# iris-ua/iris_lama

Hardware: AMD Instinct MI355X
Metric: particle-scans/sec (higher is better)
Workload: dtype f64; 1 GPU; PFSlam2D 30 particles, 1080-beam synthetic corridor log (SURVEY.md 8(d)), res 0.05 m, patch 32, l2_max 0.5, GN+Cauchy(0.15), seed 42; particles=30, beams=1080, parallelism=particle-shard x1

## Files before the change

### iris_lama_amd/csrc/lama_kernels.h

```cpp
#pragma once
#include "lama_dev.h"

namespace lama_dev {

constexpr int SM_BLOCK = 256;
constexpr int UM_BLOCK = 64;
#ifdef LAMA_TEST_SMALL_QUEUES
constexpr int LQ_SMALL = LAMA_TEST_SMALL_QUEUES, RQ_SMALL = LAMA_TEST_SMALL_QUEUES / 4;
#else
constexpr int LQ_SMALL = 1024, RQ_SMALL = 256;
#endif
constexpr int LQ_BIG = 8192, RQ_BIG = 2048;
constexpr uint32_t BF_TW_MAX_PARTICLES = 1u << 30;

template <int CTRL, int ROW_MASK>
__device__ __forceinline__ double dpp_add(double v)
{
    const uint64_t u = (uint64_t)__double_as_longlong(v);
    const uint32_t lo = (uint32_t)__builtin_amdgcn_update_dpp(0, (int)(uint32_t)u, CTRL, ROW_MASK, 0xF, false);
    const uint32_t hi = (uint32_t)__builtin_amdgcn_update_dpp(0, (int)(uint32_t)(u >> 32), CTRL, ROW_MASK, 0xF, false);
    return v + __longlong_as_double((long long)(((uint64_t)hi << 32) | lo));
}

template <int NV>
// ... 669 lines not shown
                *cell = o | (vis << 16);
                if (vis == 0) atomicOr((unsigned long long*)(occ_mask + (size_t)slot * 16 + (ci >> 6)), 1ull << (ci & 63));
                }
            }
            const int dslot = coop_slot(dm_dc, dm_dir, dm_count, (int)pv.dm_cap, changed, pidx, ERR_DM_CAP, prm.err);
            bool push = false;
            if (changed && dslot >= 0) {
                const uint64_t bit = 1ull << (ci & 63);
                uint64_t* w = dm_mask + (size_t)dslot * 16 + (ci >> 6);
                if (!(*w & bit)) atomicOr((unsigned long long*)w, (unsigned long long)bit);
                const uint32_t di = (uint32_t)dslot * 1024u + ci;
                const sv_t s = dm_sv[di];
                const bool is_obstacle = (s & SV_VALID) && (s & SV_SQMASK) == 0;
                if (is_hit) {
                    if (!is_obstacle) { dm_sv[di] = (sv_t)(SV_VALID | SV_QUEUED); dm_obs[di] = 0; push = true; }
                } else {
                    if (is_obstacle) { dm_sv[di] = SV_QUEUED; dm_obs[di] = 0; push = true; }
                }
            }
            const unsigned long long pm = __ballot(push);
            if (pm) {
                const unsigned long long pm_hit = (base == 0) ? (pm & 1ull) : 0ull;
                const unsigned long long pm_ray = pm & ~pm_hit;
                if (pm_hit) {
                    if (nl >= prm.qcap) { if (lane == 0) atomicOr(prm.err, ERR_QUEUE); }
                    else { if (push && is_hit) q_lower[nl] = q_entry(0, (int)rx, (int)ry); nl += 1; }
                }
                if (pm_ray) {
                    const int cnt = __popcll(pm_ray);
                    if (nr + (uint32_t)cnt > prm.qcap) { if (lane == 0) atomicOr(prm.err, ERR_QUEUE); }
                    else {
                        if (push && !is_hit) {
                            const int rank = __popcll(pm_ray & ((1ull << lane) - 1ull));
                            q_raise[nr + (uint32_t)rank] = q_entry(0, (int)rx, (int)ry);
                        }
                        nr += (uint32_t)cnt;
                    }
                }
            }
        }
        __builtin_amdgcn_fence(__ATOMIC_SEQ_CST, "wavefront");
    }
    if (lane == 0) {
        prm.counts[2 * p] = dm_count;
        prm.counts[2 * p + 1] = occ_count;
        prm.qsizes[2 * p] = nl;
        prm.qsizes[2 * p + 1] = nr;
        prm.stats[4 * p + 2] += ray_cells;
    }
}

#ifdef LAMA_PROFILE_BF
#ifdef LAMA_PROFILE_BF_COUNT
#define BFT(k) do { (void)tprev; } while (0)
#else
#define BFT(k) do { const uint64_t t_ = __builtin_readcyclecounter(); prof[k] += t_ - tprev; tprev = t_; } while (0)
#endif
#else
#define BFT(k) do {} while (0)
#endif
#ifdef LAMA_PROFILE_BF_MAIN
#define BFT_MAIN(k) BFT(k)
#else
#define BFT_MAIN(k) do {} while (0)
#endif
#ifdef LAMA_PROFILE_BF_FINE
#undef BFT
#undef BFT_MAIN
#define BFT(k) do {} while (0)
#define BFT_MAIN(k) do {} while (0)
#define BFF(k) do { const uint64_t t_ = __builtin_readcyclecounter(); prof[k] += t_ - tprev; tprev = t_; } while (0)
#else
#define BFF(k) do {} while (0)
#endif

constexpr int BF_DUMMY = 8;
template <int LQ, int RQ>
struct BfLds {
    uint64_t pl_e[2][4];
    uint64_t pr_e[2][4];
    uint64_t topq[2];
    uint64_t dummy[2][BF_DUMMY];
    uint32_t pl_n[2];
    uint32_t pr_n[2];
    uint32_t cmd_r;
    uint32_t cmd;
    uint32_t dc[DC_SIZE];
    uint64_t lower[LQ];
    uint64_t raise[RQ];
};
constexpr uint32_t BF_CMD_EXIT = 0xFFFFFFFFu;

__device__ __forceinline__ uint64_t lds_pop_ancestors(int lane)
{
    uint64_t anc = 0;
    if (lane < 63) for (int a = lane; a > 0; a = (a - 1) >> 1) anc |= 1ull << a;
    return anc;
}
__device__ __forceinline__ uint64_t lds_sift_topdown(uint64_t* h, const uint32_t len, const uint32_t H0, const uint64_t value, int lane, uint64_t anc)
{
    const uint32_t vprio = heap_prio(value);
    const uint32_t lim = (len - 1) / 2;
    const int d = 31 - __clz(lane + 1);
    const bool is_left = (lane & 1) != 0;
    uint32_t H = H0;
    uint32_t root_lo = (uint32_t)value, root_hi = (uint32_t)(value >> 32);
    bool stopped = false;
    while (H < lim) {
        const uint32_t idx = (H << d) + (uint32_t)lane;
        const uint32_t left = is_left ? idx : idx - 1;
        const uint32_t parent = (left - 1) >> 1;
        const bool cand = lane >= 1 && lane < 63 && parent < lim;
        const uint32_t la = cand ? left : 1u;
        const uint64_t vl = h[la], vr = h[la + 1];
        const bool take_left = heap_prio(vr) > heap_prio(vl);
        const bool step_to_me = cand && (is_left == take_left);
        const unsigned long long okm = __ballot(step_to_me);
        const bool onpath = cand && (okm & anc) == anc;
        const uint64_t mine = is_left ? vl : vr;
        const bool moves = onpath && !(heap_prio(mine) > vprio);
        const unsigned long long pathm = __ballot(onpath), mvm = __ballot(moves);
        if (moves) h[parent] = mine;
        if (mvm) {
            if (H == 0) {
                const int r1 = (mvm & 2ull) ? 1 : 2;
                root_hi = (uint32_t)__builtin_amdgcn_readlane((int)(uint32_t)(mine >> 32), r1);
                root_lo = (uint32_t)__builtin_amdgcn_readlane((int)(uint32_t)mine, r1);
            }
            const int rel = 63 - __clzll((long long)mvm);
            H = (H << (31 - __clz(rel + 1))) + (uint32_t)rel;
        }
        if (mvm != pathm) { stopped = true; break; }
    }
    LAMA_LOCKSTEP();
    if (!stopped && (len & 1) == 0 && H == (len - 2) / 2) {
        const uint64_t c = h[len - 1];
        const bool up = (uint32_t)__builtin_amdgcn_readfirstlane((int)heap_prio(c)) <= (uint32_t)__builtin_amdgcn_readfirstlane((int)vprio);
        if (up) {
            if (lane == 0) h[H] = c;
            if (H == 0) { root_lo = (uint32_t)c; root_hi = (uint32_t)(c >> 32); }
            H = len - 1;
        }
    }
    if (lane == 0) h[H] = value;
    LAMA_LOCKSTEP();
    return ((uint64_t)root_hi << 32) | root_lo;
}
__device__ __forceinline__ uint64_t lds_pop_topdown(uint64_t* h, uint32_t& size, int lane, uint64_t anc)
{
    --size;
    const uint32_t len = size;
    if (len == 0) return 0;
    return lds_sift_topdown(h, len, 0u, h[len], lane, anc);
}
__device__ __forceinline__ void lds_push(uint64_t* h, uint32_t& size, uint64_t value, bool writer)
{
    uint32_t hole = size++;
    while (hole > 0) {
        const uint32_t parent = (hole - 1) / 2;
        const uint64_t pv = h[parent];
        if (!heap_comp(pv, value)) break;
        if (writer) h[hole] = pv;
        hole = parent;
    }
    if (writer) h[hole] = value;
    LAMA_LOCKSTEP();
}

#ifdef LAMA_WAVE_SIM
struct BufRsrc { uint8_t* base; uint32_t bytes; };
__device__ __forceinline__ BufRsrc buf_make(void* p, uint32_t bytes) { return BufRsrc{(uint8_t*)p, bytes}; }
__device__ __forceinline__ uint32_t buf_load_u16(const BufRsrc& r, uint32_t off) { uint16_t v = 0; if (off <= r.bytes - 2u && off < r.bytes) std::memcpy(&v, r.base + off, 2); return v; }
__device__ __forceinline__ uint32_t buf_load_u32(const BufRsrc& r, uint32_t off) { uint32_t v = 0; if (off <= r.bytes - 4u && off < r.bytes) std::memcpy(&v, r.base + off, 4); return v; }
__device__ __forceinline__ void buf_store_u16(const BufRsrc& r, uint32_t off, uint32_t v) { if (off <= r.bytes - 2u && off < r.bytes) { const uint16_t w = (uint16_t)v; std::memcpy(r.base + off, &w, 2); } }
__device__ __forceinline__ void buf_store_u32(const BufRsrc& r, uint32_t off, uint32_t v) { if (off <= r.bytes - 4u && off < r.bytes) std::memcpy(r.base + off, &v, 4); }
__device__ __forceinline__ void buf_or_u64(const BufRsrc& r, uint32_t off, uint64_t v) { if (off <= r.bytes - 8u && off < r.bytes) { uint64_t w; std::memcpy(&w, r.base + off, 8); w |= v; std::memcpy(r.base + off, &w, 8); } }
__device__ __forceinline__ uint32_t lane_rank(unsigned long long m, int lane) { return (uint32_t)__popcll(m & ((1ull << lane) - 1ull)); }
#else
using BufRsrc = __amdgpu_buffer_rsrc_t;
__device__ __forceinline__ BufRsrc buf_make(void* p, uint32_t bytes) { return __builtin_amdgcn_make_buffer_rsrc(p, 0, (int)bytes, 0x00020000); }
__device__ __forceinline__ uint32_t buf_load_u16(BufRsrc r, uint32_t off) { return (uint32_t)(uint16_t)__builtin_amdgcn_raw_buffer_load_b16(r, (int)off, 0, 0); }
__device__ __forceinline__ uint32_t buf_load_u32(BufRsrc r, uint32_t off) { return (uint32_t)__builtin_amdgcn_raw_buffer_load_b32(r, (int)off, 0, 0); }
__device__ __forceinline__ void buf_store_u16(BufRsrc r, uint32_t off, uint32_t v) { __builtin_amdgcn_raw_buffer_store_b16((unsigned short)v, r, (int)off, 0, 0); }
__device__ __forceinline__ void buf_store_u32(BufRsrc r, uint32_t off, uint32_t v) { __builtin_amdgcn_raw_buffer_store_b32(v, r, (int)off, 0, 0); }
__device__ __forceinline__ void buf_or_u64(BufRsrc r, uint32_t off, uint64_t v) { asm volatile("s_nop 4\n\tbuffer_atomic_or_x2 %0, %1, %2, 0 offen" :: "v"(v), "v"(off), "s"(r) : "memory"); }
__device__ __forceinline__ uint32_t lane_rank(unsigned long long m, int) { return __builtin_amdgcn_mbcnt_hi((uint32_t)(m >> 32), __builtin_amdgcn_mbcnt_lo((uint32_t)m, 0u)); }
#endif
#ifdef LAMA_WIDE_DM
#define buf_load_sv buf_load_u32
#define buf_store_sv buf_store_u32
#else
#define buf_load_sv buf_load_u16
#define buf_store_sv buf_store_u16
#endif
#ifdef LAMA_WAVE_SIM
__device__ __forceinline__ uint32_t opq(uint32_t x) { return x; }
#else
__device__ __forceinline__ uint32_t opq(uint32_t x) { asm("" : "+v"(x)); return x; }
#endif
#ifdef LAMA_WAVE_SIM
__device__ __forceinline__ uint32_t pin(uint32_t x) { return x; }
#else
__device__ __forceinline__ uint32_t pin(uint32_t x) { asm volatile("" : "+v"(x)); return x; }
#endif
__device__ __forceinline__ uint32_t m_lt(uint32_t a, uint32_t b) { return opq((uint32_t)((int32_t)(opq(a) - b) >> 31)); }
__device__ __forceinline__ uint32_t m_le(uint32_t a, uint32_t b) { return ~m_lt(b, a); }
__device__ __forceinline__ uint32_t m_nz(uint32_t v) { return opq((uint32_t)((int32_t)(opq(v) | (0u - v)) >> 31)); }
__device__ __forceinline__ uint32_t m_pos(int32_t a) { return opq((uint32_t)((int32_t)(0u - (uint32_t)opq((uint32_t)a)) >> 31)); }
__device__ __forceinline__ uint32_t m_sel(uint32_t m, uint32_t a, uint32_t b) { return (a & m) | (b & ~m); }
#ifdef LAMA_WAVE_SIM
__device__ __forceinline__ uint32_t bf_mul24(uint32_t a, uint32_t b) { return a * b; }
#else
__device__ __forceinline__ uint32_t bf_mul24(uint32_t a, uint32_t b) { return __umul24(a, b); }
#endif
constexpr uint32_t BUF_OOB = 0x7FFFFFF0u;

template <int NR>
__device__ __forceinline__ void lds_pop_flat(uint64_t* h, uint32_t& size, const int lane, const uint64_t anc, uint64_t* root_out, uint64_t* dummy)
{
    --size;
    const uint32_t len = size;
    if (len == 0) return;
    const uint64_t value = h[len];
    const uint64_t tailc = h[len - 1];
    const uint32_t vprio = heap_prio(value);
    const uint32_t lim = (len - 1) >> 1;
    const int d = 31 - __clz(lane + 1);
    const uint32_t leftm = (lane & 1) ? 0xFFFFFFFFu : 0u;
    const uint32_t innerm = (lane >= 1 && lane < 63) ? 0xFFFFFFFFu : 0u;
    const uint32_t anc_lo = (uint32_t)anc, anc_hi = (uint32_t)(anc >> 32);
    uint32_t H = 0;
    uint32_t go = 0xFFFFFFFFu;
    uint64_t mine0 = 0;
    uint32_t root_child = 0;
    bool root_value = true;
#pragma unroll
    for (int r = 0; r < NR; ++r) {
        if (r > 0 && (go == 0u || ((H << 1) + 1u) >= len)) break;
        const uint32_t idx = (H << d) + (uint32_t)lane;
        const uint32_t lm1 = idx - 2u - leftm;
        const uint32_t parent = lm1 >> 1;
        const uint32_t cand = opq(innerm & go & m_lt(parent, lim));
        const uint32_t la = 1u + (lm1 & cand);
        const uint64_t vl = h[la], vr = h[la + 1];
        const uint32_t pl = (uint32_t)(vl >> 32) >> 16, pr = (uint32_t)(vr >> 32) >> 16;
        const uint32_t take_left = m_lt(pl, pr);
        const uint32_t step = opq(cand & ~(take_left ^ leftm));
        const unsigned long long okm = __ballot(step != 0u);
        const uint32_t offpath = opq((((uint32_t)okm & anc_lo) ^ anc_lo) | (((uint32_t)(okm >> 32) & anc_hi) ^ anc_hi));
        const uint32_t onpath = opq(offpath == 0u ? cand : 0u);
        const uint64_t mine = leftm ? vl : vr;
        const uint32_t pm = leftm ? pl : pr;
        const uint32_t moves = opq(onpath & m_le(pm, vprio));
        const unsigned long long pathm = __ballot(onpath != 0u), mvm = __ballot(moves != 0u);
        LAMA_LOCKSTEP();
        uint64_t* dst = moves ? h + parent : dummy;
        *dst = mine;
        if (r == 0) { mine0 = mine; root_child = opq(((lane == 1 || lane == 2) ? 0xFFFFFFFFu : 0u) & moves); root_value = (mvm & 6ull) == 0ull; }
        const int rel = 63 - __clzll((long long)(mvm | 1ull));
        const uint32_t Hn = (H << (31 - __clz(rel + 1))) + (uint32_t)rel;
        H = mvm ? Hn : H;
        go = (mvm != pathm) ? 0u : go;
        LAMA_LOCKSTEP();
    }
    const bool up = go != 0u && (len & 1u) == 0u && H == (len - 2) / 2 && heap_prio(tailc) <= vprio;
    if (__builtin_expect(up, 0)) {
        if (lane == 0) { h[H] = tailc; if (H == 0) *root_out = tailc; }
        root_value = root_value && H != 0;
        H = len - 1;
        LAMA_LOCKSTEP();
    }
    {
        const uint32_t l0 = lane == 0 ? 0xFFFFFFFFu : 0u, l3 = (lane == 3 && root_value) ? 0xFFFFFFFFu : 0u;
        uint64_t* dst = l0 ? h + H : ((l3 | root_child) ? root_out : dummy);
        const uint64_t v = root_child ? mine0 : value;
        *dst = v;
    }
    LAMA_LOCKSTEP();
}

__device__ __forceinline__ void lds_push_flat(uint64_t* heap, uint32_t& n, const uint64_t* ent, const uint32_t* cnt_p, const int lane, uint64_t* dummy)
{
    const uint32_t l4 = (uint32_t)lane & 3u;
    const uint64_t entry = ent[l4];
    const uint32_t pos = n + l4;
    const uint32_t pprio = heap_prio(heap[n >= 4 ? (pos - 1) / 2 : 0]);
    const uint32_t cnt_v = *cnt_p;
    const bool mine = (uint32_t)lane < cnt_v;
    const bool up = mine && pprio > heap_prio(entry);
    const unsigned long long upm = __ballot(up);
    const uint32_t cnt = (uint32_t)__builtin_amdgcn_readfirstlane((int)cnt_v);
    if (cnt == 0) return;
    if (__builtin_expect(n >= 4 && upm == 0ull, 1)) {
        uint64_t* dst = mine ? heap + pos : dummy;
        *dst = entry;
        n += cnt;
        LAMA_LOCKSTEP();
        return;
    }
    #pragma unroll 1
    for (uint32_t i = 0; i < cnt; ++i) lds_push(heap, n, ent[i], lane == 0);
}

__device__ __forceinline__ void lds_push_flat_n(uint64_t* heap, uint32_t& n, const uint64_t* ent, const uint32_t cnt, const int lane, uint64_t* dummy)
{
    if (cnt == 0) return;
    const uint32_t l4 = (uint32_t)lane & 3u;
    const uint64_t entry = ent[l4];
    const uint32_t pos = n + l4;
    const uint32_t pprio = heap_prio(heap[n >= 4 ? (pos - 1) / 2 : 0]);
    const bool mine = (uint32_t)lane < cnt;
    const bool up = mine && pprio > heap_prio(entry);
    const unsigned long long upm = __ballot(up);
    if (n >= 4 && upm == 0ull) {
        uint64_t* dst = mine ? heap + pos : dummy;
        *dst = entry;
        n += cnt;
        LAMA_LOCKSTEP();
        return;
    }
    #pragma unroll 1
    for (uint32_t i = 0; i < cnt; ++i) lds_push(heap, n, ent[i], lane == 0);
}

__device__ __forceinline__ bool lds_push_list(uint64_t* heap, uint32_t& n, const uint64_t* ent, const uint32_t cnt, int lane)
{
    if (!cnt) return false;
    const uint32_t l4 = (uint32_t)lane & 3u;
    const uint64_t entry = ent[l4];
    const uint32_t pos = n + l4;
    if (n >= 4) {
        const uint32_t pprio = heap_prio(heap[(pos - 1) / 2]);
        const bool mine = (uint32_t)lane < cnt;
        const bool up = mine && pprio > heap_prio(entry);
        if (__ballot(up) == 0) {
            if (mine) heap[pos] = entry;
            n += cnt;
            LAMA_LOCKSTEP();
            return true;
        }
    }
    #pragma unroll 1
    for (uint32_t i = 0; i < cnt; ++i) lds_push(heap, n, ent[i], lane == 0);
    return false;
}

#ifdef LAMA_WAVE_SIM
__device__ __forceinline__ void lds_barrier() { __syncthreads(); }
#else
__device__ __forceinline__ void lds_barrier() { asm volatile("s_waitcnt lgkmcnt(0)\n\ts_barrier" ::: "memory"); }
#endif

#ifdef LAMA_WAVE_SIM
__device__ __forceinline__ uint64_t uniform_u64(uint64_t v) { return v; }
#else
__device__ __forceinline__ uint64_t uniform_u64(uint64_t v)
{
    return ((uint64_t)(uint32_t)__builtin_amdgcn_readfirstlane((int)(uint32_t)(v >> 32)) << 32) | (uint32_t)__builtin_amdgcn_readfirstlane((int)(uint32_t)v);
}
#endif

__device__ __forceinline__ void bf_hand_over(const DevParams& prm, int p, bool from_resume)
{
    prm.slow[p] = 1;
    if (!from_resume) prm.slow_list[atomicAdd(prm.slow_n, 1u)] = (uint32_t)p;
}

template <int LQ_LDS, int RQ_LDS, bool RESUME, bool TW>
__device__ __forceinline__ void bf_particle(const DevParams& prm, const int p_any, BfLds<LQ_LDS, RQ_LDS>& sh)
{
    const int p = __builtin_amdgcn_readfirstlane(p_any);
    if (!RESUME && prm.heavy != nullptr && (prm.heavy[p] != 0 || (prm.early != nullptr && prm.early[p] != 0))) return;
    const uint32_t handed = RESUME ? prm.slow[p] : 1u;
    const int lane = threadIdx.x & 63;
    const int tid = threadIdx.x, nthreads = TW ? 2 * UM_BLOCK : UM_BLOCK;
    const PV pv = pview_w(prm, p);
    int16_t* dir = pv.dm_dir;
    sv_t* sv = pv.dm_sv;
    uint32_t* obs = pv.dm_obs;
    uint64_t* mask = pv.dm_mask;
    const uint32_t dm_cap = pv.dm_cap;
    uint64_t* g_lower = prm.q_lower + (size_t)p * prm.qcap;
    uint64_t* g_raise = prm.q_raise + (size_t)p * prm.qcap;
    int count = uload_i32(prm.counts + 2 * p);
    const uint64_t nlr = uload_u64(prm.qsizes + 2 * p);
    uint32_t nl = (uint32_t)nlr, nr = (uint32_t)(nlr >> 32);
    if (RESUME && TW) __syncthreads(); else LAMA_LOCKSTEP();
    if (RESUME && handed == 0) return;
    if (tid == 0) prm.slow[p] = 0;
    if (nl == 0 && nr == 0) return;
    if (nl + 4 > (uint32_t)LQ_LDS || nr + 4 > (uint32_t)RQ_LDS) { if (tid == 0) bf_hand_over(prm, p, RESUME); return; }

    for (int k = tid; k < DC_SIZE; k += nthreads) sh.dc[k] = DC_EMPTY;
    for (uint32_t k = tid; k < nl; k += nthreads) sh.lower[k] = g_lower[k];
    for (uint32_t k = tid; k < nr; k += nthreads) sh.raise[k] = g_raise[k];
    __syncthreads();
    const uint64_t anc = lds_pop_ancestors(lane);
    constexpr uint32_t LOWER_CAP = RESUME ? (uint32_t)LQ_LDS : (uint32_t)(LQ_LDS + RQ_LDS);
#ifndef LAMA_WAVE_SIM
    if (TW) { if (tid >= UM_BLOCK) __builtin_amdgcn_s_setprio(0); else __builtin_amdgcn_s_setprio(3); }
#endif
    if (TW && tid >= UM_BLOCK) {
        __syncthreads();
        uint32_t hnl = (uint32_t)__builtin_amdgcn_readfirstlane((int)sh.cmd), hnr = (uint32_t)__builtin_amdgcn_readfirstlane((int)sh.cmd_r);
        if (hnl == BF_CMD_EXIT) return;
#ifdef LAMA_PROFILE_BF
        uint64_t hp[3] = {0, 0, 0};
        uint64_t ht = __builtin_readcyclecounter();
        #define HFT(k) do { const uint64_t t_ = __builtin_readcyclecounter(); hp[k] += t_ - ht; ht = t_; } while (0)
#else
        #define HFT(k) do {} while (0)
#endif
        constexpr int NR = LQ_LDS > 2047 ? 3 : 2;
        #define BF_HELPER_POP(H, N, B) do { if (NR == 3 && (N) > 2047u) lds_pop_flat<3>(H, N, lane, anc, &sh.topq[B], dmy); else lds_pop_flat<2>(H, N, lane, anc, &sh.topq[B], dmy); } while (0)
        uint64_t* const dmy = sh.dummy[1] + (lane & (BF_DUMMY - 1));
        uint32_t it = 0;
        bool hstop = false;
        while (hnr > 0) {
            const uint32_t b = it & 1u;
            BF_HELPER_POP(sh.raise, hnr, b);
            lds_barrier();
            lds_push_flat(sh.raise, hnr, sh.pr_e[b], &sh.pr_n[b], lane, dmy);
            lds_push_flat(sh.lower, hnl, sh.pl_e[b], &sh.pl_n[b], lane, dmy);
            ++it;
            if (hnl + 4 > (uint32_t)LQ_LDS || (hnr > 0 && hnr + 4 > (uint32_t)RQ_LDS) || (hnr == 0 && hnl == 0)) { hstop = true; break; }
            if (hnr == 0) lds_barrier();
        }
        if (!hstop && hnl > 0) for (;;) {
            const uint32_t b = it & 1u;
            BF_HELPER_POP(sh.lower, hnl, b);
            HFT(0);
            lds_barrier();
            HFT(1);
            lds_push_flat(sh.lower, hnl, sh.pl_e[b], &sh.pl_n[b], lane, dmy);
            HFT(2);
            ++it;
            if (hnl - 1u >= LOWER_CAP - 4u) break;
        }
#ifdef LAMA_PROFILE_BF
#ifndef LAMA_PROFILE_BF_MAIN
        if (lane == 0) for (int k = 0; k < 3; ++k) prm.dbg[8 * p + 5 + k] = hp[k];
#endif
#endif
        #undef HFT
        #undef BF_HELPER_POP
        __syncthreads();
        return;
    }
    const DirCache dc{sh.dc, dir, prm.W};

    const int ddx = lane == 0 ? 1 : (lane == 2 ? -1 : 0), ddy = lane == 1 ? 1 : (lane == 3 ? -1 : 0);
    const bool is_cur = lane == 4, is_nb = lane < 4;
    uint64_t processed = 0;
    bool spill = false;
#ifdef LAMA_PROFILE_BF
    uint64_t prof[8] = {0, 0, 0, 0, 0, 0, 0, 0};
    uint64_t tprev = __builtin_readcyclecounter();
#endif

    #define BF_LOAD_A()                                                                                     \
        const int x = rx + ddx, y = ry + ddy;                                                               \
        const bool role = lane < 5;                                                                         \
        const bool inwin = (uint32_t)x < prm.WC && (uint32_t)y < prm.WC;                                    \
        const uint32_t pidx = ((uint32_t)y >> 5) * prm.W + ((uint32_t)x >> 5);                              \
        const uint32_t ci = ((uint32_t)x & 31u) | (((uint32_t)y & 31u) << 5);                               \
        int slot = (role && inwin) ? dc.lookup(pidx) : -1;                                                  \
        sv_t s = 0; uint32_t ob = 0;                                                                    \
        if (slot >= 0) { s = sv[slot * 1024 + (int)ci]; ob = obs[slot * 1024 + (int)ci]; }
    #define BF_LOAD_B()                                                                                     \
        const int ox = x + obs_x(ob), oy = y + obs_y(ob);                                                   \
        sv_t os = 0;                                                                                    \
        {                                                                                                   \
            const bool oin = role && slot >= 0 && (uint32_t)ox < prm.WC && (uint32_t)oy < prm.WC;           \
            const uint32_t opidx = ((uint32_t)oy >> 5) * prm.W + ((uint32_t)ox >> 5);                       \
            const int oslot = oin ? dc.lookup(opidx) : -1;                                                  \
            if (oslot >= 0) os = sv[oslot * 1024 + (int)(((uint32_t)ox & 31u) | (((uint32_t)oy & 31u) << 5))]; \
        }
    #define BF_POP_WITH_LOADS(H, N)                                                                         \
        BF_LOAD_A()                                                                                         \
        BFT(1);                                                                                             \
        if (TW) { --N;  } else { (void)lds_pop_topdown(H, N, lane, anc); }        \
        BF_LOAD_B()                                                                                         \
        BFT(2);

    uint64_t e_next = 0;
    uint32_t tw_it = 0;
    bool tw_running = false, tw_go = false;
    if (TW) {
        spill = nl + 4 > (uint32_t)LQ_LDS || (nr > 0 && nr + 4 > (uint32_t)RQ_LDS);
        tw_running = tw_go = !spill && (nr > 0 || nl > 0);
        if (lane == 0) { sh.cmd = tw_go ? nl : BF_CMD_EXIT; sh.cmd_r = nr; }
        if (tw_go) e_next = uniform_u64(nr > 0 ? sh.raise[0] : sh.lower[0]);
        __syncthreads();
    }
    #define BF_TW_TAIL(WAS_RAISE, NPOP, CNT_R, CNT_L, OWN_ENTRY, OWN_MASK)                                  \
        {                                                                                                   \
            const uint32_t b_ = tw_it & 1u;                                                                 \
            if (lane == 0) { sh.pr_n[b_] = (CNT_R); sh.pl_n[b_] = (CNT_L); }                                \
             \
            const uint32_t key_ = (((OWN_MASK) >> (lane & 3)) & 1u) ? ((heap_prio(OWN_ENTRY) << 2) | (uint32_t)(lane & 3)) : 0xFFFFFFFFu; \
            const uint32_t k0_ = (uint32_t)__builtin_amdgcn_readlane((int)key_, 0), k1_ = (uint32_t)__builtin_amdgcn_readlane((int)key_, 1); \
            const uint32_t k2_ = (uint32_t)__builtin_amdgcn_readlane((int)key_, 2), k3_ = (uint32_t)__builtin_amdgcn_readlane((int)key_, 3); \
            const uint32_t k01_ = k0_ < k1_ ? k0_ : k1_, k23_ = k2_ < k3_ ? k2_ : k3_;                      \
            const uint32_t kb_ = k01_ < k23_ ? k01_ : k23_;                                                 \
            const int bl_ = (int)(kb_ & 3u);                                                                \
            const uint32_t olo_ = (uint32_t)__builtin_amdgcn_readlane((int)(uint32_t)(OWN_ENTRY), bl_);     \
            const uint32_t ohi_ = (uint32_t)__builtin_amdgcn_readlane((int)(uint32_t)((OWN_ENTRY) >> 32), bl_); \
            const bool have_own_ = kb_ != 0xFFFFFFFFu;                                                      \
            BFT_MAIN(5);                                                                                    \
            lds_barrier();                                                                           \
            BFT_MAIN(7);                                                                                    \
            const bool have_root_ = (NPOP) > 0;                                                             \
            const uint64_t root_ = sh.topq[b_];                                                             \
            const bool own_wins_ = have_own_ && (!have_root_ || (kb_ >> 2) < heap_prio(root_));             \
            const uint64_t cand_ = own_wins_ ? (((uint64_t)ohi_ << 32) | olo_) : root_;                     \
            nr += (CNT_R); nl += (CNT_L);                                                                   \
            spill = nl + 4 > (uint32_t)LQ_LDS || (nr > 0 && nr + 4 > (uint32_t)RQ_LDS);                      \
            tw_running = !spill && (nr > 0 || nl > 0);                                                     \
            if (tw_running) {                                                                               \
                if ((WAS_RAISE) && nr == 0) { lds_barrier();  e_next = sh.lower[0]; }                \
                else e_next = cand_;                                                                        \
            }                                                                                               \
            ++tw_it;                                                                                        \
        }

    if (TW) {
        uint64_t* const dmy = sh.dummy[0] + (lane & (BF_DUMMY - 1));
        const BufRsrc rsv = buf_make(sv, dm_cap * SV_PATCH_BYTES), robs = buf_make(obs, dm_cap * 4096u), rmask = buf_make(mask, dm_cap * 128u);
        const bool is_oc = lane == 5;
        const uint32_t rolem = lane < 6 ? 0xFFFFFFFFu : 0u, nbm = is_nb ? 0xFFFFFFFFu : 0u, curm = is_cur ? 0xFFFFFFFFu : 0u;

        auto general_raise = [&](const uint64_t e, uint32_t& cnt_r, uint32_t& cnt_l, uint64_t& entry_r, uint32_t& rm_out) {
            const int rx = q_rx(e), ry = q_ry(e);
            BF_LOAD_A()
            BF_LOAD_B()
            if (is_nb && !inwin) atomicOr(prm.err, ERR_WINDOW);
            const bool nb = is_nb && inwin;
            const bool fresh = nb && slot < 0;
            if (__ballot(fresh)) { const int ns_ = coop_slot(dc, dir, count, (int)dm_cap, fresh, pidx, ERR_DM_CAP, prm.err); if (fresh) slot = ns_; }
            const bool nbok = nb && slot >= 0;
            if (nbok) {
                const uint64_t bit = 1ull << (ci & 63);
                if (fresh || !(s & (SV_VALID | SV_QUEUED))) atomicOr((unsigned long long*)(mask + (size_t)slot * 16 + (ci >> 6)), (unsigned long long)bit);
            }
            const bool cand = nbok && !(s & SV_QUEUED) && (s & SV_VALID);
            bool ovalid = (os & SV_VALID) != 0;
            bool clear = cand && !ovalid;
            #pragma unroll 1
            for (int i = 0; i < 3; ++i) {
                const int cxi = __builtin_amdgcn_readlane(x, i), cyi = __builtin_amdgcn_readlane(y, i);
                const bool ci_clear = __builtin_amdgcn_readlane((int)clear, i) != 0;
                if (lane > i && lane < 4 && cand && ci_clear && ox == cxi && oy == cyi) { ovalid = false; clear = true; }
            }
            const bool to_raise = cand && !ovalid, to_lower = cand && ovalid;
            const uint32_t rm = (uint32_t)__ballot(to_raise) & 15u, lm = (uint32_t)__ballot(to_lower) & 15u;
            const uint32_t below = (1u << lane) - 1u;
            entry_r = q_entry((uint32_t)(s & SV_SQMASK), x, y, obs_x(ob), obs_y(ob));
            if (to_raise) sh.pr_e[tw_it & 1u][__popc(rm & below)] = entry_r;
            if (to_lower) sh.pl_e[tw_it & 1u][__popc(lm & below)] = entry_r;
            cnt_r = (uint32_t)__popc(rm); cnt_l = (uint32_t)__popc(lm); rm_out = rm;
            if (to_raise) { sv[slot * 1024 + (int)ci] = SV_QUEUED; obs[slot * 1024 + (int)ci] = 0u; }
            if (to_lower) sv[slot * 1024 + (int)ci] = (sv_t)(s | SV_QUEUED);
            if (is_cur && slot >= 0) sv[slot * 1024 + (int)ci] = (sv_t)(s & ~SV_QUEUED);
        };

        while (tw_running && nr > 0) {
            const uint64_t e = uniform_u64(e_next);
            ++processed;
#ifdef LAMA_PROFILE_BF_COUNT
            prof[7] += 1;
#endif
            --nr;
            uint32_t cnt_r = 0, cnt_l = 0, rm = 0;
            uint64_t entry = 0;
            bool general;
            {
#ifdef LAMA_WIDE_DM
                const int rx = q_rx(e), ry = q_ry(e), eox = q_ox(e), eoy = q_oy(e);
#else
                const uint32_t elo = (uint32_t)e, ehi = (uint32_t)(e >> 32);
                const int rx = (int)(elo & 0xFFFFu), ry = (int)(elo >> 16);
                const int eox = (int)(ehi & 0xFFu) - 128, eoy = (int)((ehi >> 8) & 0xFFu) - 128;
#endif
                const int obx = rx + eox, oby = ry + eoy;
                const int x = is_oc ? obx : rx + ddx, y = is_oc ? oby : ry + ddy;
                const uint32_t mxy = (uint32_t)x > (uint32_t)y ? (uint32_t)x : (uint32_t)y;
                const uint32_t inwin = opq(mxy < prm.WC ? 0xFFFFFFFFu : 0u);
                const uint32_t pidx = bf_mul24((uint32_t)y >> 5, prm.W) + ((uint32_t)x >> 5);
                const uint32_t ci = ((uint32_t)x & 31u) | (((uint32_t)y & 31u) << 5);
                const uint32_t dv = sh.dc[dc.index(pidx & inwin)];
                const uint32_t hit = opq(inwin & ~m_nz((dv >> 15) ^ (pidx >> 3)));
                const uint32_t slotw = (dv & 0x7FFFu) - 1u;
                const uint32_t absent = opq((uint32_t)((int32_t)slotw >> 31));
                const uint32_t have = opq(rolem & hit & ~absent);
                const uint32_t coff = (slotw << 10) | ci;
                const uint32_t s = buf_load_sv(rsv, m_sel(have, coff * SV_BYTES, BUF_OOB));
                const uint32_t ob = buf_load_u32(robs, m_sel(have, coff * 4u, BUF_OOB));
                const uint32_t rare0 = (rolem & ~hit) | ((nbm | curm) & hit & absent);
                const uint32_t svalid = opq((uint32_t)((int32_t)(s << (31 - SV_VALID_BIT)) >> 31)), squeued = opq((uint32_t)((int32_t)(s << (32 - SV_VALID_BIT)) >> 31));
                const uint32_t cand = opq(nbm & svalid & ~squeued);
                const int ox = x + obs_x(ob), oy = y + obs_y(ob);
                const uint32_t same = ~(m_nz((uint32_t)(ox ^ obx)) | m_nz((uint32_t)(oy ^ oby)));
                const uint32_t other = opq(cand & ~same);
                const int ax = ox - rx, ay = oy - ry;
                const uint32_t adj = cand & ~m_nz((uint32_t)(ax * ax + ay * ay) ^ 1u);
                const unsigned long long rarem = __ballot((rare0 | adj) != 0u);
                const uint32_t cos_ = (uint32_t)__builtin_amdgcn_readlane((int)s, 5);
                uint32_t ovalid = (cos_ & SV_VALID) ? 0xFFFFFFFFu : 0u;
                general = rarem != 0ull;
                if (!general && __builtin_expect(__ballot(other != 0u) != 0ull, 0)) {
                    const uint32_t oin = opq((other != 0u && (uint32_t)ox < prm.WC && (uint32_t)oy < prm.WC) ? 0xFFFFFFFFu : 0u);
                    const uint32_t opidx = bf_mul24((uint32_t)oy >> 5, prm.W) + ((uint32_t)ox >> 5);
                    const uint32_t odv = sh.dc[dc.index(opidx & oin)];
                    const uint32_t ohit = opq((odv >> 15) == (opidx >> 3) ? oin : 0u);
                    const uint32_t oslot = (odv & 0x7FFFu) - 1u;
                    const uint32_t ooff = ((oslot << 10) | ((uint32_t)ox & 31u) | (((uint32_t)oy & 31u) << 5)) * SV_BYTES;
                    const uint32_t os2 = buf_load_sv(rsv, m_sel(ohit & ~(uint32_t)((int32_t)oslot >> 31), ooff, BUF_OOB));
                    ovalid = m_sel(other, (uint32_t)((int32_t)(os2 << (31 - SV_VALID_BIT)) >> 31), ovalid);
                    general = __ballot((oin & ~ohit) != 0u) != 0ull;
                }
                if (__builtin_expect(!general, 1)) {
                    const uint32_t to_raise = opq(cand & ~ovalid), to_lower = opq(cand & ovalid);
                    const uint32_t need_bit = nbm & ~(svalid | squeued);
                    buf_or_u64(rmask, m_sel(need_bit, ((slotw << 4) + (ci >> 6)) * 8u, BUF_OOB), 1ull << (ci & 63u));
                    const uint32_t nsv = m_sel(to_raise, (uint32_t)SV_QUEUED, m_sel(curm, s & ~(uint32_t)SV_QUEUED, s | (uint32_t)SV_QUEUED));
                    buf_store_sv(rsv, m_sel(to_raise | to_lower | curm, coff * SV_BYTES, BUF_OOB), nsv);
                    buf_store_u32(robs, m_sel(to_raise, coff * 4u, BUF_OOB), 0u);
                    const unsigned long long rmm = __ballot(to_raise != 0u), lmm = __ballot(to_lower != 0u);
                    entry = q_entry(s & SV_SQMASK, x, y, obs_x(ob), obs_y(ob));
                    const uint32_t rank_r = opq(lane_rank(rmm, lane) & 3u), rank_l = opq(lane_rank(lmm, lane) & 3u);
                    uint64_t* dst = to_raise ? &sh.pr_e[tw_it & 1u][rank_r] : (to_lower ? &sh.pl_e[tw_it & 1u][rank_l] : dmy);
                    *dst = entry;
                    cnt_r = (uint32_t)__popcll(rmm); cnt_l = (uint32_t)__popcll(lmm); rm = (uint32_t)rmm & 15u;
                }
            }
            if (__builtin_expect(general, 0)) general_raise(e, cnt_r, cnt_l, entry, rm);
#ifndef LAMA_WAVE_SIM
            cnt_r = (uint32_t)__builtin_amdgcn_readfirstlane((int)cnt_r); cnt_l = (uint32_t)__builtin_amdgcn_readfirstlane((int)cnt_l);
            rm = (uint32_t)__builtin_amdgcn_readfirstlane((int)rm);
#endif
            {
                const uint32_t b_ = tw_it & 1u;
                uint32_t* np = lane == 0 ? &sh.pr_n[b_] : (lane == 1 ? &sh.pl_n[b_] : (uint32_t*)dmy);
                *np = lane == 0 ? cnt_r : cnt_l;
                lds_barrier();
                const uint64_t root_ = sh.topq[b_];
                const uint32_t rlo = (uint32_t)__builtin_amdgcn_readfirstlane((int)(uint32_t)root_), rhi = (uint32_t)__builtin_amdgcn_readfirstlane((int)(uint32_t)(root_ >> 32));
                const bool have_root = nr > 0;
                uint64_t cand_ = ((uint64_t)rhi << 32) | rlo;
                if (cnt_r > 0) {
                    uint32_t key = (lane < 4 && ((rm >> lane) & 1u)) ? ((heap_prio(entry) << 2) | (uint32_t)lane) : 0xFFFFFFFFu;
                    uint32_t blo = (uint32_t)entry, bhi = (uint32_t)(entry >> 32);
#define BF_QUAD_MIN(CTRL)                                                                                              \
                    {                                                                                                  \
                        const uint32_t k2 = (uint32_t)__builtin_amdgcn_update_dpp((int)key, (int)key, CTRL, 0xF, 0xF, false); \
                        const uint32_t l2 = (uint32_t)__builtin_amdgcn_update_dpp((int)blo, (int)blo, CTRL, 0xF, 0xF, false); \
                        const uint32_t h2 = (uint32_t)__builtin_amdgcn_update_dpp((int)bhi, (int)bhi, CTRL, 0xF, 0xF, false); \
                        const bool t_ = k2 < key;                                                                      \
                        key = t_ ? k2 : key; blo = t_ ? l2 : blo; bhi = t_ ? h2 : bhi;                                 \
                    }
                    BF_QUAD_MIN(0xB1)
                    BF_QUAD_MIN(0x4E)
#undef BF_QUAD_MIN
                    const uint32_t okey = (uint32_t)__builtin_amdgcn_readfirstlane((int)key);
                    const uint32_t olo = (uint32_t)__builtin_amdgcn_readfirstlane((int)blo), ohi = (uint32_t)__builtin_amdgcn_readfirstlane((int)bhi);
                    if (!have_root || (okey >> 2) < (rhi >> 16)) cand_ = ((uint64_t)ohi << 32) | olo;
                }
                nr += cnt_r; nl += cnt_l;
                spill = nl + 4 > (uint32_t)LQ_LDS || (nr > 0 && nr + 4 > (uint32_t)RQ_LDS);
                tw_running = !spill && (nr > 0 || nl > 0);
                if (tw_running) {
                    if (nr == 0) { lds_barrier();  e_next = uniform_u64(sh.lower[0]); }
                    else e_next = cand_;
                }
                ++tw_it;
            }
            __builtin_amdgcn_fence(__ATOMIC_SEQ_CST, "wavefront");
        }
    }
    while (!TW && nr > 0) {
        if (!TW && (nl + 4 > (uint32_t)LQ_LDS || nr + 4 > (uint32_t)RQ_LDS)) { spill = true; break; }
        const uint64_t e = TW ? e_next : sh.raise[0];
        const int rx = q_rx(e), ry = q_ry(e);
        ++processed;
#ifdef LAMA_PROFILE_BF_COUNT
        prof[7] += 1;
#endif
        BF_POP_WITH_LOADS(sh.raise, nr)
        if (is_nb && !inwin) atomicOr(prm.err, ERR_WINDOW);
        const bool nb = is_nb && inwin;
        const bool fresh = nb && slot < 0;
        if (__ballot(fresh)) { const int ns_ = coop_slot(dc, dir, count, (int)dm_cap, fresh, pidx, ERR_DM_CAP, prm.err); if (fresh) slot = ns_; }
        const bool nbok = nb && slot >= 0;
        if (nbok) {
            const uint64_t bit = 1ull << (ci & 63);
            if (fresh || !(s & (SV_VALID | SV_QUEUED))) atomicOr((unsigned long long*)(mask + (size_t)slot * 16 + (ci >> 6)), (unsigned long long)bit);
        }
        const bool cand = nbok && !(s & SV_QUEUED) && (s & SV_VALID);
        bool ovalid = (os & SV_VALID) != 0;
        bool clear = cand && !ovalid;
        #pragma unroll 1
        for (int i = 0; i < 3; ++i) {
            const int cxi = __builtin_amdgcn_readlane(x, i), cyi = __builtin_amdgcn_readlane(y, i);
            const bool ci_clear = __builtin_amdgcn_readlane((int)clear, i) != 0;
            if (lane > i && lane < 4 && cand && ci_clear && ox == cxi && oy == cyi) { ovalid = false; clear = true; }
        }
        const bool to_raise = cand && !ovalid;
        const bool to_lower = cand && ovalid;
        uint32_t rw_cnt_r = 0, rw_cnt_l = 0, rw_rm = 0;
        uint64_t rw_entry_r = 0;
        if (TW) {
            const uint32_t rm = (uint32_t)__ballot(to_raise) & 15u, lm = (uint32_t)__ballot(to_lower) & 15u;
            const uint32_t below = (1u << lane) - 1u;
            rw_entry_r = q_entry((uint32_t)(s & SV_SQMASK), x, y);
            if (to_raise) sh.pr_e[tw_it & 1u][__popc(rm & below)] = rw_entry_r;
            if (to_lower) sh.pl_e[tw_it & 1u][__popc(lm & below)] = q_entry((uint32_t)(s & SV_SQMASK), x, y, obs_x(ob), obs_y(ob));
            rw_cnt_r = (uint32_t)__popc(rm); rw_cnt_l = (uint32_t)__popc(lm); rw_rm = rm;
        }
        #pragma unroll 1
        for (int i = 0; !TW && i < 4; ++i) {
            const bool r_i = __builtin_amdgcn_readlane((int)to_raise, i) != 0, l_i = __builtin_amdgcn_readlane((int)to_lower, i) != 0;
            if (r_i || l_i) {
                const uint32_t prio = (uint32_t)__builtin_amdgcn_readlane((int)(s & SV_SQMASK), i);
                const int ex = __builtin_amdgcn_readlane(x, i), ey = __builtin_amdgcn_readlane(y, i);
                const uint32_t eo = (uint32_t)__builtin_amdgcn_readlane((int)ob, i);
                if (r_i) lds_push(sh.raise, nr, q_entry(prio, ex, ey), lane == 0);
                else lds_push(sh.lower, nl, q_entry(prio, ex, ey, obs_x(eo), obs_y(eo)), lane == 0);
            }
        }
        if (to_raise) { sv[slot * 1024 + (int)ci] = SV_QUEUED; obs[slot * 1024 + (int)ci] = 0u; }
        if (to_lower) sv[slot * 1024 + (int)ci] = (sv_t)(s | SV_QUEUED);
        if (is_cur && slot >= 0) sv[slot * 1024 + (int)ci] = (sv_t)(s & ~SV_QUEUED);
        if (TW) BF_TW_TAIL(true, nr, rw_cnt_r, rw_cnt_l, rw_entry_r, rw_rm)
        __builtin_amdgcn_fence(__ATOMIC_SEQ_CST, "wavefront");
    }

    constexpr bool PAIR = TW;
    if (TW || !spill) {
        if (!TW) { tw_running = nl > 0; if (tw_running) e_next = uniform_u64(sh.lower[0]); }
        BFT(7);
        uint64_t* const dmy = sh.dummy[0] + (lane & (BF_DUMMY - 1));
        const BufRsrc rsv = buf_make(sv, dm_cap * SV_PATCH_BYTES), robs = buf_make(obs, dm_cap * 4096u), rmask = buf_make(mask, dm_cap * 128u);
        const bool is_oc = lane == 5, role = lane < 6;
        const uint32_t rolem = role ? 0xFFFFFFFFu : 0u, nbm = is_nb ? 0xFFFFFFFFu : 0u, curm = is_cur ? 0xFFFFFFFFu : 0u;

        auto general_pop = [&](const uint64_t e, bool& over_out, uint64_t& entry_out) -> uint32_t {
            over_out = false; entry_out = 0;
// ... 955 lines not shown
```

Before: 16820 particle-scans/s.

## Plan next heap pop before barrier and commit after push in helper wave

```diff
diff --git a/iris_lama_amd/csrc/lama_kernels.h b/iris_lama_amd/csrc/lama_kernels.h
--- a/iris_lama_amd/csrc/lama_kernels.h
+++ b/iris_lama_amd/csrc/lama_kernels.h
@@ -995,6 +995,122 @@
     for (uint32_t i = 0; i < cnt; ++i) lds_push(heap, n, ent[i], lane == 0);
 }
 
+template <int NR>
+struct PopPlan {
+    uint64_t mine[NR];
+    uint32_t pm[NR];
+    uint32_t parent[NR];
+    unsigned long long pathm[NR];
+    uint64_t value0;
+    uint32_t hend;
+    uint32_t n;
+};
+constexpr uint32_t BF_PLAN_OFF = 0x7FFFFFFFu;
+
+template <int NR>
+__device__ __forceinline__ void lds_pop_plan(const uint64_t* h, const uint32_t n, const int lane, const uint64_t anc, PopPlan<NR>& pl)
+{
+    pl.n = 0; pl.hend = 0; pl.value0 = 0;
+#pragma unroll
+    for (int r = 0; r < NR; ++r) { pl.mine[r] = 0; pl.pm[r] = BF_PLAN_OFF; pl.parent[r] = 0; pl.pathm[r] = 0ull; }
+    if (n < 4u) return;
+    const uint32_t len = n - 1u;
+    pl.value0 = h[len];
+    const uint32_t lim = (len - 1u) >> 1;
+    const int d = 31 - __clz(lane + 1);
+    const uint32_t leftm = (lane & 1) ? 0xFFFFFFFFu : 0u;
+    const uint32_t innerm = (lane >= 1 && lane < 63) ? 0xFFFFFFFFu : 0u;
+    const uint32_t anc_lo = (uint32_t)anc, anc_hi = (uint32_t)(anc >> 32);
+    uint32_t H = 0;
+#pragma unroll
+    for (int r = 0; r < NR; ++r) {
+        if (r > 0 && (pl.pathm[r - 1] == 0ull || ((H << 1) + 1u) >= len)) break;
+        const uint32_t idx = (H << d) + (uint32_t)lane;
+        const uint32_t lm1 = idx - 2u - leftm;
+        const uint32_t parent = lm1 >> 1;
+        const uint32_t cand = opq(innerm & m_lt(parent, lim));
+        const uint32_t la = 1u + (lm1 & cand);
+        const uint64_t vl = h[la], vr = h[la + 1];
+        const uint32_t pl_ = (uint32_t)(vl >> 32) >> 16, pr_ = (uint32_t)(vr >> 32) >> 16;
+        const uint32_t take_left = m_lt(pl_, pr_);
+        const uint32_t step = opq(cand & ~(take_left ^ leftm));
+        const unsigned long long okm = __ballot(step != 0u);
+        const uint32_t offpath = opq((((uint32_t)okm & anc_lo) ^ anc_lo) | (((uint32_t)(okm >> 32) & anc_hi) ^ anc_hi));
+        const uint32_t onpath = opq(offpath == 0u ? cand : 0u);
+        const unsigned long long pathm = __ballot(onpath != 0u);
+        pl.mine[r] = leftm ? vl : vr;
+        pl.pm[r] = m_sel(onpath, leftm ? pl_ : pr_, BF_PLAN_OFF);
+        pl.parent[r] = parent;
+        pl.pathm[r] = pathm;
+        const int rel = 63 - __clzll((long long)(pathm | 1ull));
+        const uint32_t Hn = (H << (31 - __clz(rel + 1))) + (uint32_t)rel;
+        H = pathm ? Hn : H;
+    }
+    pl.hend = H;
+    pl.n = n;
+}
+
+template <int NR>
+__device__ __forceinline__ void lds_push_planned(uint64_t* heap, uint32_t& n, const uint64_t* ent, const uint32_t* cnt_p, const int lane, uint64_t* dummy,
+                                                 const PopPlan<NR>& pl, uint32_t* why, uint64_t* value)
+{
+    const uint32_t l4 = (uint32_t)lane & 3u;
+    const uint64_t entry = ent[l4];
+    const uint32_t pos = n + l4;
+    const uint32_t pprio = heap_prio(heap[n >= 4 ? (pos - 1) / 2 : 0]);
+    const uint32_t cnt_v = *cnt_p;
+    const bool mine = (uint32_t)lane < cnt_v;
+    const bool up = mine && pprio > heap_prio(entry);
+    const unsigned long long upm = __ballot(up);
+    const uint32_t cnt = (uint32_t)__builtin_amdgcn_readfirstlane((int)cnt_v);
+    *why = 1u;
+    if (__builtin_expect(n >= 4 && upm == 0ull, 1)) {
+        uint64_t* dst = mine ? heap + pos : dummy;
+        *dst = entry;
+        const uint64_t src = cnt ? entry : pl.value0;
+        const int sl = cnt ? (int)cnt - 1 : 0;
+        const uint32_t vlo = (uint32_t)__builtin_amdgcn_readlane((int)(uint32_t)src, sl), vhi = (uint32_t)__builtin_amdgcn_readlane((int)(uint32_t)(src >> 32), sl);
+        *value = ((uint64_t)vhi << 32) | vlo;
+        *why = (pl.n == n && 2u * pl.hend + 1u >= n + cnt - 1u) ? 0u : 2u;
+        n += cnt;
+        LAMA_LOCKSTEP();
+        return;
+    }
+    #pragma unroll 1
+    for (uint32_t i = 0; i < cnt; ++i) lds_push(heap, n, ent[i], lane == 0);
+}
+
+template <int NR>
+__device__ __forceinline__ void lds_pop_commit(uint64_t* h, uint32_t& size, const int lane, const PopPlan<NR>& pl, const uint64_t value, uint64_t* root_out, uint64_t* dummy)
+{
+    --size;
+    const uint32_t vprio = heap_prio(value);
+    uint32_t H = 0;
+    uint32_t go = 0xFFFFFFFFu;
+    uint32_t root_child = 0;
+    bool root_value = true;
+#pragma unroll
+    for (int r = 0; r < NR; ++r) {
+        if (r > 0 && (go == 0u || pl.pathm[r] == 0ull)) break;
+        const uint32_t moves = opq(m_le(pl.pm[r], vprio));
+        const unsigned long long mvm = __ballot(moves != 0u);
+        uint64_t* dst = moves ? h + pl.parent[r] : dummy;
+        *dst = pl.mine[r];
+        if (r == 0) { root_child = opq(((lane == 1 || lane == 2) ? 0xFFFFFFFFu : 0u) & moves); root_value = (mvm & 6ull) == 0ull; }
+        const int rel = 63 - __clzll((long long)(mvm | 1ull));
+        const uint32_t Hn = (H << (31 - __clz(rel + 1))) + (uint32_t)rel;
+        H = mvm ? Hn : H;
+        go = (mvm != pl.pathm[r]) ? 0u : go;
+    }
+    {
+        const uint32_t l0 = lane == 0 ? 0xFFFFFFFFu : 0u, l3 = (lane == 3 && root_value) ? 0xFFFFFFFFu : 0u;
+        uint64_t* dst = l0 ? h + H : ((l3 | root_child) ? root_out : dummy);
+        const uint64_t v = root_child ? pl.mine[0] : value;
+        *dst = v;
+    }
+    LAMA_LOCKSTEP();
+}
+
 __device__ __forceinline__ void lds_push_flat_n(uint64_t* heap, uint32_t& n, const uint64_t* ent, const uint32_t cnt, const int lane, uint64_t* dummy)
 {
     if (cnt == 0) return;
@@ -1100,35 +1216,57 @@
 #ifdef LAMA_PROFILE_BF
         uint64_t hp[3] = {0, 0, 0};
         uint64_t ht = __builtin_readcyclecounter();
+#ifdef LAMA_PROFILE_BF_COUNT
+        #define HFT(k) do { (void)ht; } while (0)
+        #define HCNT(why) do { hp[why] += 1; } while (0)
+#else
         #define HFT(k) do { const uint64_t t_ = __builtin_readcyclecounter(); hp[k] += t_ - ht; ht = t_; } while (0)
+        #define HCNT(why) do {} while (0)
+#endif
 #else
         #define HFT(k) do {} while (0)
+        #define HCNT(why) do {} while (0)
 #endif
         constexpr int NR = LQ_LDS > 2047 ? 3 : 2;
         #define BF_HELPER_POP(H, N, B) do { if (NR == 3 && (N) > 2047u) lds_pop_flat<3>(H, N, lane, anc, &sh.topq[B], dmy); else lds_pop_flat<2>(H, N, lane, anc, &sh.topq[B], dmy); } while (0)
         uint64_t* const dmy = sh.dummy[1] + (lane & (BF_DUMMY - 1));
         uint32_t it = 0;
         bool hstop = false;
-        while (hnr > 0) {
-            const uint32_t b = it & 1u;
-            BF_HELPER_POP(sh.raise, hnr, b);
-            lds_barrier();
-            lds_push_flat(sh.raise, hnr, sh.pr_e[b], &sh.pr_n[b], lane, dmy);
-            lds_push_flat(sh.lower, hnl, sh.pl_e[b], &sh.pl_n[b], lane, dmy);
-            ++it;
-            if (hnl + 4 > (uint32_t)LQ_LDS || (hnr > 0 && hnr + 4 > (uint32_t)RQ_LDS) || (hnr == 0 && hnl == 0)) { hstop = true; break; }
-            if (hnr == 0) lds_barrier();
-        }
-        if (!hstop && hnl > 0) for (;;) {
-            const uint32_t b = it & 1u;
-            BF_HELPER_POP(sh.lower, hnl, b);
-            HFT(0);
-            lds_barrier();
-            HFT(1);
-            lds_push_flat(sh.lower, hnl, sh.pl_e[b], &sh.pl_n[b], lane, dmy);
-            HFT(2);
-            ++it;
-            if (hnl - 1u >= LOWER_CAP - 4u) break;
+        PopPlan<NR> plan;
+        uint32_t why = 0;
+        uint64_t value = 0;
+        if (hnr > 0) {
+            BF_HELPER_POP(sh.raise, hnr, 0u);
+            for (;;) {
+                const uint32_t b = it & 1u;
+                lds_pop_plan<NR>(sh.raise, hnr, lane, anc, plan);
+                lds_barrier();
+                lds_push_planned<NR>(sh.raise, hnr, sh.pr_e[b], &sh.pr_n[b], lane, dmy, plan, &why, &value);
+                lds_push_flat(sh.lower, hnl, sh.pl_e[b], &sh.pl_n[b], lane, dmy);
+                ++it;
+                if (hnl + 4 > (uint32_t)LQ_LDS || (hnr > 0 && hnr + 4 > (uint32_t)RQ_LDS) || (hnr == 0 && hnl == 0)) { hstop = true; break; }
+                if (hnr == 0) { lds_barrier(); break; }
+                HCNT(why);
+                if (__builtin_expect(why == 0u, 1)) lds_pop_commit<NR>(sh.raise, hnr, lane, plan, value, &sh.topq[it & 1u], dmy);
+                else BF_HELPER_POP(sh.raise, hnr, it & 1u);
+            }
+        }
+        if (!hstop && hnl > 0) {
+            BF_HELPER_POP(sh.lower, hnl, it & 1u);
+            for (;;) {
+                const uint32_t b = it & 1u;
+                lds_pop_plan<NR>(sh.lower, hnl, lane, anc, plan);
+                HFT(0);
+                lds_barrier();
+                HFT(1);
+                lds_push_planned<NR>(sh.lower, hnl, sh.pl_e[b], &sh.pl_n[b], lane, dmy, plan, &why, &value);
+                ++it;
+                if (hnl - 1u >= LOWER_CAP - 4u) break;
+                HCNT(why);
+                if (__builtin_expect(why == 0u, 1)) lds_pop_commit<NR>(sh.lower, hnl, lane, plan, value, &sh.topq[it & 1u], dmy);
+                else BF_HELPER_POP(sh.lower, hnl, it & 1u);
+                HFT(2);
+            }
         }
 #ifdef LAMA_PROFILE_BF
 #ifndef LAMA_PROFILE_BF_MAIN
@@ -1136,6 +1274,7 @@
 #endif
 #endif
         #undef HFT
+        #undef HCNT
         #undef BF_HELPER_POP
         __syncthreads();
         return;
```

Measured after the change: 14780 particle-scans/s. 0.879x the previous value.
